# importZL/semantic_segmentation

Hardware: AMD Instinct MI355X
Metric: images/sec (fwd+bwd) U-Net 256x256 bs=32 per GPU (higher is better)
Workload: dtype f16; 1 GPU; unet.UNet(1,2) 256x256 fwd+bwd, CE+Dice loss, batch 32/GPU (BASELINE configs[1]); global_batch=32, parallelism=dp1, dice=per-rank

## Files before the change

include/gsseg.h:

```cpp
#ifndef GSSEG_H
#define GSSEG_H

#include <stdint.h>

#ifdef __cplusplus
extern "C" {
#endif

#define GS_ABI_VERSION 52

enum GsDtype { GS_F16 = 0, GS_BF16 = 1 };
enum GsStatus { GS_OK = 0, GS_EINVAL = -1, GS_ELAUNCH = -2, GS_EUNSUPPORTED = -3 };
enum GsAct { GS_ACT_NONE = 0, GS_ACT_RELU = 1, GS_ACT_LEAKY02 = 2, GS_ACT_TANH = 3 };

#define GS_MAX_TAPS 64

typedef struct GsConvGeom {
    int32_t N, IH, IW, Cin, in_pix_stride, in_coff;
    int32_t OHg, OWg, Cout;
    int32_t OH, OW, out_pix_stride, out_coff;
    int32_t isy, isx, osy, osx, ooy, oox;
    int32_t ntaps;
    int32_t tap_dy[GS_MAX_TAPS], tap_dx[GS_MAX_TAPS];
    int32_t tap_w[GS_MAX_TAPS];
    int32_t Dg, Din, Dout, isz, osz, ooz;
    int32_t tap_dz[GS_MAX_TAPS];
} GsConvGeom;

const char* gs_last_error(void);
int gs_abi_version(void);

int gs_conv_igemm_mtiles(const GsConvGeom* g);
// ... 100 lines not shown
                     int res_pix_stride, int res_coff, void* dz, int NB, int D, int H, int W, int C, int dtype,
                     void* stream);

int gs_maxpool2x2_fwd(const void* z, int z_pix_stride, int z_coff, void* zp, int N, int H, int W, int C, int dtype,
                      void* stream);
int gs_maxpool2x2_fwd_pair(const void* z_hi, const void* z_lo, int z_pix_stride, void* zp_hi, void* zp_lo, int zp_pix_stride, int N, int H,
                           int W, int C, int dtype, void* stream);

int gs_colsum(const void* t, int pix_stride, int coff, int N, int H, int W, int y0, int x0, int h, int w, int C,
              float gscale, float* ws, float* out, int dtype, void* stream);

int gs_head1x1_bn_fwd(const void* y_conv, const float* bn_scale, const float* bn_shift, int act, const float* w,
                      const float* bias, float* logits, int N, int H, int W, int Cout, int dtype, void* stream);
int gs_head1x1_bn_wgrad(const void* y_conv, const float* bn_scale, const float* bn_shift, int act, const float* w,
                        const float* dl, float* dw, float* db, float* ws, int N, int H, int W, int Cout, float gscale,
                        int dtype, void* stream);

int gs_bn_act_bwd_reduce_head(const void* y, const float* dl, const float* w_head, int ncls, const float* scale,
                              const float* shift, const float* mean, const float* invstd, int act, float* partials, int N,
                              int H, int W, int C, int dtype, void* stream);
int gs_bn_act_bwd_apply_head(const void* y, const float* dl, const float* w_head, int ncls, const float* scale,
                             const float* shift, const float* mean, const float* invstd, const float* c1, const float* c2,
                             int act, void* dy, int N, int H, int W, int C, int dtype, void* stream);

int gs_bn_partials_colsum(const float* partials, int ntiles, int Cfull, int coff, int C, float gscale, float* out,
                          void* stream);

int gs_pack_weight(const float* w, void* w_fwd, void* w_dgrad, int Cout, int Cin, int taps, int transposed,
                   int dtype, void* stream);

typedef struct GsPackDesc {
    const float* w;
    void* w_fwd;
    void* w_dgrad;
    int32_t Cout, Cin, taps, transposed;
} GsPackDesc;
int gs_pack_weight_multi(int n, const GsPackDesc* descs, int dtype, void* stream);
int gs_unpack_wgrad(const float* dw, float* grad, int A, int B, int taps, int transposed, float gscale, void* stream);

int64_t gs_fake_postprocess_ws_floats(int N);
int gs_fake_postprocess(const float* x, float* out, float* ws, const float* gamma_lut, int N, int64_t hw, void* stream);

int64_t gs_isic_fake_trans_ws_bytes(int planes, int64_t hw);
int gs_isic_fake_trans(const float* x, float* out, void* ws, int N, int C, int H, int W, int equalize_on, int bits,
                       int sharpness_on, float sharp_r1, float sharp_r2, int autocontrast_on, int saturation_on, float sat_r1,
                       float sat_r2, void* stream);
// ... 165 lines not shown
```

semantic_segmentation_amd/_lib.py:

```python
from __future__ import annotations

import ctypes
import os
import subprocess
from ctypes import POINTER, c_char_p, c_double, c_float, c_int, c_int32, c_int64, c_void_p

_HERE = os.path.dirname(os.path.abspath(__file__))
LIB_PATH = os.environ.get("GSSEG_LIB", os.path.join(_HERE, "libgsseg_hip.so"))
CSRC = os.path.join(_HERE, "csrc")

GS_F16, GS_BF16 = 0, 1
ACT_NONE, ACT_RELU, ACT_LEAKY02, ACT_TANH = 0, 1, 2, 3
GS_MAX_TAPS = 64
ABI_VERSION = 52


class GsConvGeom(ctypes.Structure):
    _fields_ = [(n, c_int32) for n in (
        "N", "IH", "IW", "Cin", "in_pix_stride", "in_coff", "OHg", "OWg", "Cout", "OH", "OW",
        "out_pix_stride", "out_coff", "isy", "isx", "osy", "osx", "ooy", "oox", "ntaps")] + [
        ("tap_dy", c_int32 * GS_MAX_TAPS), ("tap_dx", c_int32 * GS_MAX_TAPS), ("tap_w", c_int32 * GS_MAX_TAPS)] + [
        (n, c_int32) for n in ("Dg", "Din", "Dout", "isz", "osz", "ooz")] + [("tap_dz", c_int32 * GS_MAX_TAPS)]


class GsPackDesc(ctypes.Structure):
    _fields_ = [("w", c_void_p), ("w_fwd", c_void_p), ("w_dgrad", c_void_p)] + [
        (n, c_int32) for n in ("Cout", "Cin", "taps", "transposed")]


GS_SEG_MAX = 4


class GsSegPackDesc(ctypes.Structure):
    _fields_ = [("w", c_void_p), ("pack", c_void_p)] + [(n, c_int32) for n in ("Cout", "Cin", "taps", "transposed", "nseg")] + [
        ("kind", c_int32 * GS_SEG_MAX), ("ci0", c_int32 * GS_SEG_MAX), ("len", c_int32 * GS_SEG_MAX)]


# ... 60 lines not shown
    "gs_bn_bwd_tiles_used": (c_int, [c_int, c_int, c_int, c_int]),
    "gs_bn_act_bwd_reduce": (c_int, [_P, _P, c_int, c_int, _P, _P, c_int, _P, c_float, _F, _F, _F, _F, c_int, _F]
                             + [c_int] * 5 + [c_void_p]),
    "gs_bn_bwd_coeffs": (c_int, [_F, c_int, c_int, c_double, c_float, _F, _F, _F, _F, c_void_p]),
    "gs_bn_act_bwd_apply": (c_int, [_P, _P, c_int, c_int, _P, _P, c_int, _P, c_float, _F, _F, _F, _F, _F, _F, c_int,
                                    c_int, _P]
                            + [c_int] * 5 + [c_void_p]),
    "gs_maxpool3d_fwd": (c_int, [_P, c_int, c_int, _P] + [c_int] * 6 + [c_void_p]),
    "gs_maxpool2x2_fwd": (c_int, [_P, c_int, c_int, _P] + [c_int] * 5 + [c_void_p]),
    "gs_maxpool2x2_fwd_pair": (c_int, [_P, _P, c_int, _P, _P, c_int] + [c_int] * 5 + [c_void_p]),
    "gs_maxpool3d_bwd": (c_int, [_P, c_int, c_int, _P, _P, c_int, c_int, _P] + [c_int] * 6 + [c_void_p]),
    "gs_colsum": (c_int, [_P, c_int, c_int] + [c_int] * 8 + [c_float, _F, _F, c_int, c_void_p]),
    "gs_stem_bn_bwd_wgrad": (c_int, [_P, _P, c_int, c_int, _F, _F, _F, _F, _F, _F, _F, c_int, _F, _F, c_int, c_int, c_int,
                                     c_float, c_int, c_void_p]),
    "gs_stem_stats": (c_int, [_F, _F, _F, _F, c_int, c_int, c_int, c_void_p]),
    "gs_stem_bwd_onepass": (c_int, [_F, _P, _P, c_int, c_int, c_int, _F, _F, c_int, c_int, c_int, c_int, c_void_p]),
    "gs_stem_bwd_finalize": (c_int, [_F, _F, _F, _F, _F, _F, _F, c_int, c_float, _F, _F, _F, c_int, c_int, c_int, c_void_p]),
    "gs_stem_fwd_bn": (c_int, [_F, _F, _F, _F, c_int, _P, c_int, c_int, c_int, c_int, c_void_p]),
    "gs_stem_bwd_tiles": (c_int, [c_int, c_int, c_int]),
    "gs_head1x1_bn_fwd": (c_int, [_P, _F, _F, c_int, _F, _F, _F] + [c_int] * 5 + [c_void_p]),
    "gs_head1x1_bn_wgrad": (c_int, [_P, _F, _F, c_int, _F, _F, _F, _F, _F] + [c_int] * 4 + [c_float, c_int, c_void_p]),
    "gs_bn_act_bwd_reduce_head": (c_int, [_P, _F, _F, c_int, _F, _F, _F, _F, c_int, _F] + [c_int] * 5 + [c_void_p]),
    "gs_bn_act_bwd_apply_head": (c_int, [_P, _F, _F, c_int, _F, _F, _F, _F, _F, _F, c_int, _P] + [c_int] * 5 + [c_void_p]),
    "gs_bn_partials_colsum": (c_int, [_F, c_int, c_int, c_int, c_int, c_float, _F, c_void_p]),
    "gs_pack_weight": (c_int, [_F, _P, _P, c_int, c_int, c_int, c_int, c_int, c_void_p]),
    "gs_pack_weight_multi": (c_int, [c_int, POINTER(GsPackDesc), c_int, c_void_p]),
    "gs_unpack_wgrad": (c_int, [_F, _F, c_int, c_int, c_int, c_int, c_float, c_void_p]),
    "gs_upconv_merge_pack": (c_int, [_F, _F, _F, _F, _P, _P, _F, c_int, c_int, c_int, c_void_p]),
    "gs_fake_postprocess_ws_floats": (c_int64, [c_int]),
    "gs_isic_fake_trans_ws_bytes": (c_int64, [c_int, c_int64]),
    "gs_isic_fake_trans": (c_int, [_F, _F, _P, c_int, c_int, c_int, c_int, c_int, c_int, c_int, c_float, c_float, c_int, c_int,
                                   c_float, c_float, c_void_p]),
    "gs_fake_postprocess": (c_int, [_F, _F, _F, _F, c_int, c_int64, c_void_p]),
    "gs_upconv8_image_fwd": (c_int, [_P, c_int, c_int, _P, c_int, _F, _F, _P] + [c_int] * 7 + [c_void_p]),
    "gs_upconv8_image_wgrad_ok": (c_int, [c_int, c_int]),
    "gs_upconv8_image_wgrad_ws_floats": (c_int64, [c_int] * 4),
    "gs_upconv8_image_wgrad": (c_int, [_P, c_int, _P, c_int, _F, _F] + [c_int] * 5 + [c_void_p]),
    "gs_upconv_split_wgrad": (c_int, [_F, _F, _F, _F, _F, c_float, _F, _F, _F, _F, c_int, c_int, c_void_p]),
    "gs_upconv_split_wgrad_det": (c_int, [_F, _F, _F, _F, _F, c_float, _F, _F, _F, _F, _F, c_int, c_int, c_void_p]),
    "gs_upconv_split_wgrad_ws_floats": (c_int64, [c_int, c_int]),
    "gs_upconv_split_wgrad_parts_ok": (c_int, [c_int, c_int]),
    "gs_upconv_split_wgrad_parts": (c_int, [_F, c_int, c_int64, _F, _F, _F, _F, c_float, _F, _F, _F, _F, _F, c_int, c_int, c_void_p]),
    "gs_nchw_to_nhwc": (c_int, [_F, _P] + [c_int] * 7 + [c_void_p]),
    "gs_nhwc_to_nchw": (c_int, [_P, c_int, c_int, _F] + [c_int] * 4 + [c_float, c_int, c_void_p]),
    "gs_seg_loss_fwd": (c_int, [_F, _P, c_int, c_int, c_int, c_int, _F, _F, c_void_p]),
    "gs_seg_loss_bwd": (c_int, [_F, _P, _F, _F, c_float, _F, c_int, c_int, c_int, c_int, c_void_p]),
# ... 90 lines not shown
```

semantic_segmentation_amd/csrc/bn.hip:

```cpp
#include <stdlib.h>

#include "common.hpp"

namespace {

constexpr int RED_SLICES = 64;

__global__ __launch_bounds__(256) void reduce_partials_stage1(const float* __restrict__ part, int ntiles, int C,
                                                              int tiles_per_slice, double* __restrict__ out1) {
    __shared__ double red[2][8][32];
    const int cl = threadIdx.x & 31, tl = threadIdx.x >> 5;
    const int c = blockIdx.x * 32 + cl;
    const int t0 = blockIdx.y * tiles_per_slice, t1 = min(ntiles, t0 + tiles_per_slice);
    double s1 = 0.0, s2 = 0.0;
    if (c < C) {
        for (int tt = t0 + tl; tt < t1; tt += 8) {
            s1 += (double)part[((int64_t)tt * 2 + 0) * C + c];
            s2 += (double)part[((int64_t)tt * 2 + 1) * C + c];
        }
    }
    red[0][tl][cl] = s1;
    red[1][tl][cl] = s2;
    __syncthreads();
    if (tl == 0 && c < C) {
// ... 43 lines not shown
    shift[c] = bt - (float)mean * sc;
    mean_out[c] = (float)mean;
    invstd_out[c] = invstd;
    if (running_mean) running_mean[c] = (1.f - momentum) * running_mean[c] + momentum * (float)mean;
    if (running_var) {
        const double unb = count > 1.0 ? var * (count / (count - 1.0)) : var;
        running_var[c] = (1.f - momentum) * running_var[c] + momentum * (float)unb;
    }
}

__global__ void bn_eval_coeffs_kernel(int C, const float* gamma, const float* beta, const float* rm, const float* rv,
                                      float eps, float* scale, float* shift, float* mean, float* invstd) {
    const int c = blockIdx.x * blockDim.x + threadIdx.x;
    if (c >= C) return;
    const float is = 1.f / sqrtf(rv[c] + eps);
    const float sc = (gamma ? gamma[c] : 1.f) * is;
    scale[c] = sc;
    shift[c] = (beta ? beta[c] : 0.f) - rm[c] * sc;
    mean[c] = rm[c];
    invstd[c] = is;
}

template <typename T>
__global__ __launch_bounds__(256) void bn_bwd_coeffs_kernel(const T* __restrict__ s, int nslices, int C, double count,
                                                            float gscale, float* dgamma, float* dbeta, float* c1, float* c2) {
    double s1, s2;
    sum_slices_32x8(s, nslices, C, s1, s2);
    const int c = blockIdx.x * 32 + (threadIdx.x & 31);
    if (c >= C || threadIdx.x >= 32) return;
    if (dbeta) dbeta[c] = (float)(s1 * gscale);
    if (dgamma) dgamma[c] = (float)(s2 * gscale);
    c1[c] = (float)(s1 / count);
    c2[c] = (float)(s2 / count);
}

static int bn_traversal() {
    static const int v = getenv("GSSEG_BN_REV") ? atoi(getenv("GSSEG_BN_REV")) : 3;
    return v;
}

struct ApplyArgs {
    const unsigned short* y;
    const float* scale;
    const float* shift;
    unsigned short* z;
    unsigned short* zp;
    const uint8_t* keep;
    float keep_scale;
    int act, N, H, W, C, zs, zc;
    int rev;
};

template <int DT, bool POOL, bool GENERIC>
__global__ __launch_bounds__(256) void bn_act_apply_kernel(const ApplyArgs a) {
    const float slope = a.act == GS_ACT_RELU ? 0.f : (a.act == GS_ACT_LEAKY02 ? 0.2f : 1.f);
    auto fwd_a = [&](float v) __attribute__((always_inline)) { return GENERIC ? act_fwd(v, a.act) : (v > 0.f ? v : v * slope); };
// ... 64 lines not shown
__device__ __forceinline__ float mul_rn(float a, float b) {
    float r;
    asm("v_mul_f32 %0, %1, %2" : "=v"(r) : "v"(a), "v"(b));
    return r;
}

struct BwdArgs {
    const unsigned short* y;
    const unsigned short* dza;
    const unsigned short* dzp;
    const unsigned short* dzb;
    const uint8_t* keep;
    float keep_scale;
    int act_b;
    const float *scale, *shift, *mean, *invstd, *c1, *c2;
    float* partials;
    unsigned short* dy;
    int sa, ca, act, bn, N, H, W, C;
    int tile_units;
    int rev;
    const float* head_dl;
    const float* head_w;
    int head_n;
};

template <int DT, bool POOL, bool APPLY, bool GENERIC, int HEAD = 0, bool EXTRA = true, bool RN = false>
__global__ __launch_bounds__(256) void bn_act_bwd_kernel(const BwdArgs a) {
    static_assert(!HEAD || (!POOL && !GENERIC), "the head source: plain pixels, slope-family activation");
    static_assert(!(RN && GENERIC), "the rounded slope product belongs to the slope family");
    auto mul_g = [&](float g, float d) __attribute__((always_inline)) { return RN ? mul_rn(g, d) : g * d; };
    constexpr int NH = HEAD ? HEAD : 1;
    constexpr int HEAD_CHUNK = 2048;
    __shared__ float hdl[HEAD ? NH * HEAD_CHUNK : 1];
    __shared__ float red[2][256 * 8 / 8][8];
    const float slope_a = a.act == GS_ACT_RELU ? 0.f : (a.act == GS_ACT_LEAKY02 ? 0.2f : 1.f);
    const float slope_b = a.act_b == GS_ACT_RELU ? 0.f : (a.act_b == GS_ACT_LEAKY02 ? 0.2f : 1.f);
    auto grad_a = [&](float v) __attribute__((always_inline)) { return GENERIC ? act_grad(v, a.act) : (v > 0.f ? 1.f : slope_a); };
    auto grad_b = [&](float v) __attribute__((always_inline)) { return GENERIC ? act_grad(v, a.act_b) : (v > 0.f ? 1.f : slope_b); };
    auto fwd_a = [&](float v) __attribute__((always_inline)) { return GENERIC ? act_fwd(v, a.act) : (v > 0.f ? v : v * slope_a); };
    const int nch = a.C >> 3;
    const int PH = POOL ? (a.H + 1) / 2 : a.H, PW = POOL ? (a.W + 1) / 2 : a.W;
    const int units = a.N * PH * PW;
    const int lanes_per_unit = nch < 256 ? nch : 256;
    const int unit_lanes = 256 / lanes_per_unit;
    const int chl = threadIdx.x % lanes_per_unit, ul = threadIdx.x / lanes_per_unit;
    const int tile = a.rev ? (int)(gridDim.x - 1 - blockIdx.x) : (int)blockIdx.x;
    const int u0 = tile * a.tile_units;
    int u1 = u0 + a.tile_units < units ? u0 + a.tile_units : units;
    if (ul >= unit_lanes) u1 = u0;
    constexpr int UNR = 4;

// ... 1 lines not shown
        const bool ch_ok = ch < nch;
        const int c0 = ch_ok ? ch * 8 : 0;
        if (!ch_ok) u1 = u0;
        float sc[8], sh[8], mu[8], is[8], k1[8], k2[8];
#pragma unroll
        for (int i = 0; i < 8; ++i) {
            sc[i] = a.scale ? a.scale[c0 + i] : 1.f;
            sh[i] = a.shift ? a.shift[c0 + i] : 0.f;
            mu[i] = a.mean ? a.mean[c0 + i] : 0.f;
            is[i] = a.invstd ? a.invstd[c0 + i] : 1.f;
            k1[i] = (APPLY && a.c1) ? a.c1[c0 + i] : 0.f;
            k2[i] = (APPLY && a.c2) ? a.c2[c0 + i] : 0.f;
        }
        float s1[8], s2[8];
#pragma unroll
        for (int i = 0; i < 8; ++i) { s1[i] = 0.f; s2[i] = 0.f; }
        float hw[NH][8];
        if (HEAD) {
#pragma unroll
            for (int k = 0; k < NH; ++k)
#pragma unroll
                for (int i = 0; i < 8; ++i) hw[k][i] = k < a.head_n ? a.head_w[k * a.C + c0 + i] : 0.f;
        }
        const int HWp = a.H * a.W;

        if (!POOL) {
            const int tile_end = u0 + a.tile_units < units ? u0 + a.tile_units : units;
            const int chunk = HEAD ? HEAD_CHUNK : (tile_end - u0 > 0 ? tile_end - u0 : 1);
            for (int cb = u0; cb < tile_end; cb += chunk) {
            const int ce = cb + chunk < tile_end ? cb + chunk : tile_end;
            if (HEAD) {
                __syncthreads();
                for (int i = threadIdx.x; i < ce - cb; i += 256) {
                    const int p = cb + i, n = p / HWp, hwp = p - n * HWp;
#pragma unroll
                    for (int q = 0; q < NH; ++q) hdl[q * HEAD_CHUNK + i] = q < a.head_n ? a.head_dl[((int64_t)n * a.head_n + q) * HWp + hwp] : 0.f;
                }
                __syncthreads();
            }
            const int ue = ce < u1 ? ce : u1;
            for (int ub = cb + ul; ub < ue; ub += unit_lanes * UNR) {
                uint4 ry[UNR], rg[UNR], rb[UNR];
                uint2 rk[UNR];
                bool ok[UNR];
                float hd[UNR][NH];
#pragma unroll
// ... 21 lines not shown
                    unpack8<DT>(rg[k], g);
                    unpack8<DT>(rb[k], gb);
                    if (HEAD) {
#pragma unroll
                        for (int i = 0; i < 8; ++i) {
                            float t = hd[k][0] * hw[0][i];
#pragma unroll
                            for (int q = 1; q < NH; ++q) t += hd[k][q] * hw[q][i];
                            g[i] = t;
                        }
                    }
                    if (EXTRA && a.keep) {
                        const unsigned int kw[2] = {rk[k].x, rk[k].y};
#pragma unroll
                        for (int i = 0; i < 8; ++i) g[i] *= ((kw[i >> 2] >> (8 * (i & 3))) & 0xffu) ? a.keep_scale : 0.f;
                    }
#pragma unroll
                    for (int i = 0; i < 8; ++i) {
                        const float v = yv[i] * sc[i] + sh[i];
                        const float gh = mul_g(g[i], grad_a(v)) + ((EXTRA && a.dzb) ? mul_g(gb[i], grad_b(v)) : 0.f);
                        const float xh = (yv[i] - mu[i]) * is[i];
                        if (APPLY) out[i] = a.bn ? sc[i] * (gh - k1[i] - xh * k2[i]) : gh;
                        else { s1[i] += gh; s2[i] += gh * xh; }
                    }
                    if (APPLY) st16(a.dy + pix * a.C + c0, pack8<DT>(out));
                }
            }
            }
        } else {
            const int PH2 = a.H / 2, PW2 = a.W / 2;
            for (int u = u0 + ul; u < u1; u += unit_lanes) {
                const int px = u % PW;
                const int r = u / PW;
                const int py = r % PH;
                const int n = r / PH;
                uint4 ry[4], rg[4];
                bool ok[4];
                int64_t pixk[4];
#pragma unroll
                for (int k = 0; k < 4; ++k) {
                    const int yy = 2 * py + (k >> 1), xx = 2 * px + (k & 1);
                    ok[k] = yy < a.H && xx < a.W;
                    pixk[k] = ((int64_t)n * a.H + (yy < a.H ? yy : a.H - 1)) * a.W + (xx < a.W ? xx : a.W - 1);
                    ry[k] = *reinterpret_cast<const uint4*>(a.y + pixk[k] * a.C + c0);
                    rg[k] = a.dza ? *reinterpret_cast<const uint4*>(a.dza + pixk[k] * a.sa + a.ca + c0) : make_uint4(0, 0, 0, 0);
                }
// ... 37 lines not shown
                        const float v = yv[k][i] * sc[i] + sh[i];
                        const float gh = mul_g(gz, grad_a(v));
                        const float xh = (yv[k][i] - mu[i]) * is[i];
                        if (APPLY) out[i] = a.bn ? sc[i] * (gh - k1[i] - xh * k2[i]) : gh;
                        else { s1[i] += gh; s2[i] += gh * xh; }
                    }
                    if (APPLY) st16(a.dy + pixk[k] * a.C + c0, pack8<DT>(out));
                }
            }
        }
        if (!APPLY) {
            __syncthreads();
#pragma unroll
            for (int i = 0; i < 8; ++i) { red[0][threadIdx.x][i] = s1[i]; red[1][threadIdx.x][i] = s2[i]; }
            __syncthreads();
            const int nv = lanes_per_unit * 8;
            for (int v = threadIdx.x; v < 2 * nv; v += 256) {
                const int st = v >= nv ? 1 : 0, idx = v - st * nv;
                const int cl = idx >> 3, i = idx & 7;
                if (ch - chl + cl >= nch) continue;
                float tsum = 0.f;
                for (int k = 0; k < unit_lanes; ++k) tsum += red[st][k * lanes_per_unit + cl][i];
                a.partials[(int64_t)tile * 2 * a.C + st * a.C + (ch - chl + cl) * 8 + i] = tsum;
            }
        }
    }
}

template <int DT>
__global__ __launch_bounds__(256) void colsum_stage1(const unsigned short* __restrict__ t, int ps, int coff,
                                                     int64_t npix, int C, int64_t pix_per_block, float* ws,
                                                     int H, int W, int y0, int x0, int h, int w) {
    __shared__ float red[256][8];
    const int nch = C >> 3;
    const int lpu = nch < 256 ? nch : 256, ulanes = 256 / lpu;
    const int chl = threadIdx.x % lpu, ul = threadIdx.x / lpu;
    const int64_t p0 = (int64_t)blockIdx.x * pix_per_block;
    int64_t p1 = p0 + pix_per_block < npix ? p0 + pix_per_block : npix;
    if (ul >= ulanes) p1 = p0;
    for (int ch = chl; ch - chl < nch; ch += lpu) {
        float s[8];
#pragma unroll
        for (int i = 0; i < 8; ++i) s[i] = 0.f;
        if (ch >= nch) p1 = p0;
        for (int64_t p = p0 + ul; p < p1; p += ulanes) {
            float v[8];
            const int xx = (int)(p % w);
            const int64_t r = p / w;
            const int yy = (int)(r % h);
            const int64_t n = r / h;
            const int64_t pp = (n * H + y0 + yy) * W + x0 + xx;
            unpack8<DT>(*reinterpret_cast<const uint4*>(t + pp * ps + coff + ch * 8), v);
#pragma unroll
            for (int i = 0; i < 8; ++i) s[i] += v[i];
        }
        __syncthreads();
#pragma unroll
        for (int i = 0; i < 8; ++i) red[threadIdx.x][i] = s[i];
        __syncthreads();
        for (int v = threadIdx.x; v < lpu * 8; v += 256) {
            const int cl = v >> 3, i = v & 7;
            if (ch - chl + cl >= nch) continue;
            float tt = 0.f;
            for (int k = 0; k < ulanes; ++k) tt += red[k * lpu + cl][i];
            ws[(int64_t)blockIdx.x * C + (ch - chl + cl) * 8 + i] = tt;
        }
    }
}
__global__ __launch_bounds__(256) void colsum_stage2(const float* ws, int nblocks, int C, float gscale, float* out) {
    __shared__ double red[8][32];
    const int cl = threadIdx.x & 31, tl = threadIdx.x >> 5;
    const int c = blockIdx.x * 32 + cl;
    double s = 0.0;
    if (c < C) {
        double a[8] = {0, 0, 0, 0, 0, 0, 0, 0};
        int i = tl;
        for (; i + 56 < nblocks; i += 64) {
            float v[8];
#pragma unroll
            for (int u = 0; u < 8; ++u) v[u] = ws[(int64_t)(i + 8 * u) * C + c];
#pragma unroll
            for (int u = 0; u < 8; ++u) a[u] += (double)v[u];
        }
        for (; i < nblocks; i += 8) a[0] += (double)ws[(int64_t)i * C + c];
        s = ((a[0] + a[1]) + (a[2] + a[3])) + ((a[4] + a[5]) + (a[6] + a[7]));
    }
    red[tl][cl] = s;
    __syncthreads();
    if (tl == 0 && c < C) {
        double t = 0.0;
#pragma unroll
        for (int i = 0; i < 8; ++i) t += red[i][cl];
        out[c] = (float)(t * gscale);
    }
}

__global__ __launch_bounds__(256) void partials_colsum_stage1(const float* __restrict__ part, int ntiles, int Cfull, int coff, int C,
                                                              int tiles_per_slice, double* __restrict__ out1) {
    __shared__ double red[8][32];
    const int cl = threadIdx.x & 31, tl = threadIdx.x >> 5;
    const int c = blockIdx.x * 32 + cl;
    const int t0 = blockIdx.y * tiles_per_slice, t1 = min(ntiles, t0 + tiles_per_slice);
    double s1 = 0.0;
    if (c < C)
        for (int tt = t0 + tl; tt < t1; tt += 8) s1 += (double)part[(int64_t)tt * 2 * Cfull + coff + c];
    red[tl][cl] = s1;
    __syncthreads();
    if (tl == 0 && c < C) {
        double a = 0.0;
#pragma unroll
        for (int i = 0; i < 8; ++i) a += red[i][cl];
        out1[(int64_t)blockIdx.y * C + c] = a;
    }
}

template <typename T>
__global__ __launch_bounds__(256) void partials_colsum_final(const T* __restrict__ s, int n, int64_t stride, int C, float gscale,
// ... 126 lines not shown
    const int PH = pool ? (a.H + 1) / 2 : a.H, PW = pool ? (a.W + 1) / 2 : a.W;
    const int64_t units = (int64_t)a.N * PH * PW;
    const int ntiles_max = gs_bn_bwd_tiles(a.N, a.H, a.W);
    a.tile_units = (int)cdiv64(units, ntiles_max);
    if (a.tile_units < 1) a.tile_units = 1;
    const int ntiles = (int)cdiv64(units, a.tile_units);
    if (ntiles_out) *ntiles_out = ntiles;
    const bool generic = a.act == GS_ACT_TANH || (a.dzb && a.act_b == GS_ACT_TANH);
    const bool leaky = !generic && (a.act == GS_ACT_LEAKY02 || (a.dzb && a.act_b == GS_ACT_LEAKY02));
#define LAUNCH(DT, G, R)                                                                                \
    do {                                                                                                \
        if (pool) {                                                                                     \
            if (apply) bn_act_bwd_kernel<DT, true, true, G, 0, true, R><<<ntiles, 256, 0, s>>>(a);      \
            else bn_act_bwd_kernel<DT, true, false, G, 0, true, R><<<ntiles, 256, 0, s>>>(a);           \
        } else if (a.dzb != nullptr || a.keep != nullptr) {                                             \
            if (apply) bn_act_bwd_kernel<DT, false, true, G, 0, true, R><<<ntiles, 256, 0, s>>>(a);     \
            else bn_act_bwd_kernel<DT, false, false, G, 0, true, R><<<ntiles, 256, 0, s>>>(a);          \
        } else {                                                                                        \
            if (apply) bn_act_bwd_kernel<DT, false, true, G, 0, false, R><<<ntiles, 256, 0, s>>>(a);    \
            else bn_act_bwd_kernel<DT, false, false, G, 0, false, R><<<ntiles, 256, 0, s>>>(a);         \
        }                                                                                               \
    } while (0)
    if (a.head_dl != nullptr) {
#define LAUNCH_HEAD(DT, NC, R)                                                                          \
    do {                                                                                                \
        if (apply) bn_act_bwd_kernel<DT, false, true, false, NC, false, R><<<ntiles, 256, 0, s>>>(a);   \
        else bn_act_bwd_kernel<DT, false, false, false, NC, false, R><<<ntiles, 256, 0, s>>>(a);        \
    } while (0)
#define LAUNCH_HEAD_N(DT, R) do { if (a.head_n <= 2) LAUNCH_HEAD(DT, 2, R); else LAUNCH_HEAD(DT, 4, R); } while (0)
        if (dtype == GS_F16) { if (leaky) LAUNCH_HEAD_N(GS_F16, true); else LAUNCH_HEAD_N(GS_F16, false); }
        else { if (leaky) LAUNCH_HEAD_N(GS_BF16, true); else LAUNCH_HEAD_N(GS_BF16, false); }
#undef LAUNCH_HEAD_N
#undef LAUNCH_HEAD
        return 0;
    }
    if (dtype == GS_F16) { if (generic) LAUNCH(GS_F16, true, false); else if (leaky) LAUNCH(GS_F16, false, true); else LAUNCH(GS_F16, false, false); }
    else { if (generic) LAUNCH(GS_BF16, true, false); else if (leaky) LAUNCH(GS_BF16, false, true); else LAUNCH(GS_BF16, false, false); }
#undef LAUNCH
    return 0;
}

extern "C" int gs_bn_bwd_tiles_used(int N, int H, int W, int pooled) {
    const int PH = pooled ? (H + 1) / 2 : H, PW = pooled ? (W + 1) / 2 : W;
    const int64_t units = (int64_t)N * PH * PW;
    const int ntiles_max = gs_bn_bwd_tiles(N, H, W);
    int64_t tu = cdiv64(units, ntiles_max);
    if (tu < 1) tu = 1;
    return (int)cdiv64(units, tu);
}

// ... 65 lines not shown
    GS_CHECK_ARG(dtype == GS_F16 || dtype == GS_BF16, "%s: bad dtype", who);
    GS_CHECK_ARG((int64_t)N * H * W < 2147483647LL, "%s: more than 2^31 pixels", who);
    GS_CHECK_ARG(act == GS_ACT_NONE || act == GS_ACT_RELU || act == GS_ACT_LEAKY02, "%s: activation %d not supported", who, act);
    GS_CHECK_ARG(scale && shift && mean && invstd, "%s: needs the BatchNorm coefficients", who);
    a.y = (const unsigned short*)y; a.head_dl = dl; a.head_w = w_head; a.head_n = ncls;
    a.scale = scale; a.shift = shift; a.mean = mean; a.invstd = invstd; a.act = act; a.bn = 1;
    a.N = N; a.H = H; a.W = W; a.C = C;
    return GS_OK;
}

extern "C" int gs_bn_act_bwd_reduce_head(const void* y, const float* dl, const float* w_head, int ncls, const float* scale,
                                         const float* shift, const float* mean, const float* invstd, int act, float* partials,
                                         int N, int H, int W, int C, int dtype, void* stream) {
    BwdArgs a{};
    int rc = bn_head_args("gs_bn_act_bwd_reduce_head", a, y, dl, w_head, ncls, scale, shift, mean, invstd, act, N, H, W, C, dtype);
    if (rc) return rc;
    GS_CHECK_ARG(partials != nullptr, "gs_bn_act_bwd_reduce_head: null partials");
    a.partials = partials;
    launch_bwd(a, false, dtype, (hipStream_t)stream, nullptr);
    GS_CHECK_LAUNCH("gs_bn_act_bwd_reduce_head");
    return GS_OK;
}

extern "C" int gs_bn_act_bwd_apply_head(const void* y, const float* dl, const float* w_head, int ncls, const float* scale,
                                        const float* shift, const float* mean, const float* invstd, const float* c1,
                                        const float* c2, int act, void* dy, int N, int H, int W, int C, int dtype, void* stream) {
    BwdArgs a{};
    int rc = bn_head_args("gs_bn_act_bwd_apply_head", a, y, dl, w_head, ncls, scale, shift, mean, invstd, act, N, H, W, C, dtype);
    if (rc) return rc;
    GS_CHECK_ARG(dy && c1 && c2, "gs_bn_act_bwd_apply_head: null pointer");
    a.c1 = c1; a.c2 = c2; a.dy = (unsigned short*)dy;
    launch_bwd(a, true, dtype, (hipStream_t)stream, nullptr);
    GS_CHECK_LAUNCH("gs_bn_act_bwd_apply_head");
    return GS_OK;
}

extern "C" int gs_bn_partials_colsum(const float* partials, int ntiles, int Cfull, int coff, int C, float gscale, float* out,
                                     void* stream) {
    GS_CHECK_ARG(partials && out && ntiles > 0 && Cfull > 0 && C > 0 && coff >= 0 && coff + C <= Cfull,
                 "gs_bn_partials_colsum: bad arguments");
    hipStream_t s = (hipStream_t)stream;
    if (ntiles <= direct_tiles()) {
        partials_colsum_final<float><<<cdiv(C, 32), 256, 0, s>>>(partials + coff, ntiles, (int64_t)2 * Cfull, C, gscale, out);
    } else {
        int slices = ntiles < RED_SLICES ? ntiles : RED_SLICES;
        const int tps = cdiv(ntiles, slices);
// ... 29 lines not shown
```

semantic_segmentation_amd/ops.py:

```python
from __future__ import annotations

import collections
import ctypes
import os
from typing import List, Optional, Sequence, Tuple

import torch

from . import _lib
from ._lib import ACT_NONE, GS_BF16, GS_F16, GsConvGeom

DTYPES = {"f16": (GS_F16, torch.float16), "bf16": (GS_BF16, torch.bfloat16)}


def dt_code(t: torch.Tensor) -> int:
    if t.dtype == torch.float16:
        return GS_F16
    if t.dtype == torch.bfloat16:
        return GS_BF16
    raise TypeError(f"expected a float16/bfloat16 tensor, got {t.dtype}")


def _p(t: Optional[torch.Tensor]):
    return None if t is None else t.data_ptr()
# ... 783 lines not shown
              ncls, float(gscale), dt_code(y_conv), _stream())


def bn_act_bwd_reduce_head(y, dl, w_head, scale, shift, mean, invstd, act, partials):
    _dev(y)
    _f32(dl, "dl"); _f32(w_head, "w_head"); _f32(partials, "partials")
    N, H, W, C = y.shape
    ncls = dl.shape[1]
    if tuple(dl.shape) != (N, ncls, H, W) or w_head.numel() != ncls * C or not (dl.is_contiguous() and w_head.is_contiguous()):
        raise ValueError("bn_act_bwd_reduce_head: dl [N,ncls,H,W] and w_head [ncls,C] contiguous fp32")
    _lib.call("gs_bn_act_bwd_reduce_head", _p(y), _p(dl), _p(w_head), ncls, _p(scale), _p(shift), _p(mean), _p(invstd), act,
              _p(partials), N, H, W, C, dt_code(y), _stream())


def bn_act_bwd_apply_head(y, dl, w_head, scale, shift, mean, invstd, c1, c2, act, dy):
    _dev(y)
    _f32(dl, "dl"); _f32(w_head, "w_head")
    N, H, W, C = y.shape
    ncls = dl.shape[1]
    if tuple(dl.shape) != (N, ncls, H, W) or w_head.numel() != ncls * C or not (dl.is_contiguous() and w_head.is_contiguous()):
        raise ValueError("bn_act_bwd_apply_head: dl [N,ncls,H,W] and w_head [ncls,C] contiguous fp32")
    _lib.call("gs_bn_act_bwd_apply_head", _p(y), _p(dl), _p(w_head), ncls, _p(scale), _p(shift), _p(mean), _p(invstd),
              _p(c1), _p(c2), act, _p(dy), N, H, W, C, dt_code(y), _stream())


def bn_partials_colsum(partials, ntiles, Cfull, coff, C, gscale, out):
    _f32(partials, "partials"); _f32(out, "out")
    if partials.numel() < bn_partials_numel(ntiles, Cfull) or out.numel() < C:
        raise ValueError("bn_partials_colsum: buffer too small")
    _lib.call("gs_bn_partials_colsum", _p(partials), ntiles, Cfull, coff, C, float(gscale), _p(out), _stream())


def colsum(t, pix_stride, coff, N, H, W, y0, x0, h, w, C, gscale, ws, out):
    _f32(ws, "ws"); _f32(out, "out")
    if ws.numel() < 1024 * C:
        raise ValueError("colsum: workspace must hold 1024*C floats")
    _lib.call("gs_colsum", _p(t), pix_stride, coff, N, H, W, y0, x0, h, w, C, float(gscale), _p(ws), _p(out),
              dt_code(t), _stream())


def pack_weight(w, w_fwd, w_dgrad, transposed: bool):
    _dev(w)
    _f32(w, "weight")
    if transposed:
        Cin, Cout = w.shape[0], w.shape[1]
    else:
# ... 564 lines not shown
```

semantic_segmentation_amd/unet/unet_engine.py:

```python
from __future__ import annotations

import functools
import math
import os
import warnings
from typing import Callable, Dict, List, Optional

import torch

from .. import ops
from .._lib import ACT_NONE, ACT_RELU
from ..engine_common import ParamIndex, _flush_nbt, bn_coeffs, compute_dtype, pack_key, pack_reuse_allowed

FOLD_BN_INFERENCE = os.environ.get("GSSEG_FOLD_BN", "1") != "0"
WGRAD_SIDE_STREAM = os.environ.get("GSSEG_WGRAD_STREAM", "0") != "0"
FUSED_STEM_BWD = os.environ.get("GSSEG_STEM_BWD_FUSED", "1") != "0"
FUSED_STEM_FWD = os.environ.get("GSSEG_STEM_FWD_FUSED", "1") != "0"
FUSED_HEAD_FWD = os.environ.get("GSSEG_HEAD_FWD_FUSED", "1") != "0"
FUSED_HEAD_BWD = os.environ.get("GSSEG_HEAD_BWD_FUSED", "1") != "0"
FUSED_UP_BIAS_GRAD = os.environ.get("GSSEG_UP_BIAS_FUSED", "1") != "0"


class _ConvRec:
    __slots__ = ("name", "wkey", "bnkey", "inp", "inp_is_image", "y", "coef", "geom", "cin", "cout", "h", "w",
                 "wd", "train_stats", "inp_stride", "z", "tap_sums", "wide")


class _UpRec:
    __slots__ = ("name", "zin", "cat", "geom_bwd", "geom_wg", "wd", "cin", "cout", "h", "w", "H2", "W2", "pt", "pl")


STREAM_SMALL_CONV = os.environ.get("GSSEG_STREAM_CONV", "1") != "0"


@functools.lru_cache(maxsize=4096)
def stream_conv(N, h, w, cin, cout):
    M = N * h * w
    if not STREAM_SMALL_CONV or M > 8192 or cin % 64 or cout % 32:
        return False
    tiles = (-(-w // 32)) * (-(-h // 8)) if w >= 24 else (-(-w // 16)) * (-(-h // 16))
    if N * tiles * (-(-cout // 64)) > 128:
        return False
# ... 760 lines not shown
        dw_arena = torch.zeros(max(tot_w, 1), dtype=torch.float32, device=dev)
        wg_ws = empty(wg_need, dtype=torch.float32)
        arena_off = [0]

        def dw_take(numel):
            a = arena_off[0]
            arena_off[0] = a + numel
            return dw_arena[a:a + numel]
        npart = 0
        for i in range(5):
            npart = max(npart, ops.bn_partials_numel(ops.bn_bwd_tiles(N, hs[i], ws_[i]), C[i]))
            if i == 0:
                npart = max(npart, ops.bn_partials_numel(ops.stem_bwd_tiles(N, hs[i], ws_[i]), 64))
            if i < 4 and ops.USE_HALO_CONV:
                npart = max(npart, ops.bn_partials_numel(ops.conv3x3_mtiles(N, hs[i], ws_[i], 2 * C[i]), 2 * C[i]))
                if N * hs[i] * ws_[i] <= 8192:
                    npart = max(npart, ops.bn_partials_numel(-(-(N * hs[i] * ws_[i]) // 16), 2 * C[i]))
        partials = empty(npart, dtype=torch.float32)
        col_ws = empty(1024 * 1024, dtype=torch.float32)

        z_last = ctx["z_last"]
        dl = (dlogits.contiguous().float() * S)
        wout = params["outc.conv.weight"]
        dwo = galloc("outc.conv.weight", wout, zero=True)
        dbo = galloc("outc.conv.bias", params["outc.conv.bias"], zero=True)
        head_src = None
        wout_c = wout.detach().contiguous()
        rlast = recs["up4.conv.3"]
        if z_last is None:
            ops.head1x1_bn_wgrad(rlast.y, rlast.coef[0], rlast.coef[1], ACT_RELU, wout_c, dl, dwo, dbo, gscale=inv_s)
        if FUSED_HEAD_BWD and wout.shape[0] <= 4 and dl.is_contiguous():
            head_src = (dl, wout_c)
            dz = None
            if z_last is not None:
                ops.conv_smallcout_bwd(z_last, wout_c, dl, None, dwo, dbo, gscale=inv_s)
        elif 4 < wout.shape[0] <= 64:
            dz = empty(N, H, W, 64)
            ops.head1x1_wide_bwd(z_last, wout_c.reshape(wout.shape[0], 64), dl, dz, dwo, dbo, gscale=inv_s)
        elif wout.shape[0] > 64:
            dzs = torch.zeros((N, H, W, 64), dtype=torch.float32, device=dev)
            for g0 in range(0, wout.shape[0], 4):
                g1 = min(g0 + 4, wout.shape[0])
                dzg = empty(N, H, W, 64)
                ops.conv_smallcout_bwd(z_last, wout_c[g0:g1].contiguous(), dl[:, g0:g1].contiguous(), dzg, dwo[g0:g1], dbo[g0:g1],
                                       gscale=inv_s)
                dzs += dzg
            dz = dzs.to(tdt)
        else:
            dz = empty(N, H, W, 64)
            if z_last is not None:
                ops.conv_smallcout_bwd(z_last, wout_c, dl, dz, dwo, dbo, gscale=inv_s)
            else:
                ops.conv_smallcout_bwd(None, wout_c, dl, dz, None, None)
        emit("outc.conv.weight", dwo)
        emit("outc.conv.bias", dbo)

        def conv_stage_bwd(rec: _ConvRec, dz_a, sa, ca, dzp, need_dinp: bool, colsum=None, head=None):
            h, w, cin, cout = rec.h, rec.w, rec.cin, rec.cout
            coef = rec.coef
            pooled = dzp is not None
            if rec.y is None:
                wst = params[rec.wkey].detach().contiguous()
                done = False
                if not need_dinp and not pooled and head is None:
                    nts = ops.stem_bwd_tiles(N, h, w)
                    sws = empty(nts * 576, dtype=torch.float32)
                    s1p = empty(nts * 64, dtype=torch.float32)
                    if ops.stem_bwd_onepass(rec.inp, rec.z, dz_a, sa, ca, ACT_RELU, s1p, sws, z_stride=rec.z.shape[3]):
                        dgamma = galloc(rec.bnkey + ".weight", params[rec.bnkey + ".weight"])
                        dbeta = galloc(rec.bnkey + ".bias", params[rec.bnkey + ".bias"])
                        dw = galloc(rec.wkey, params[rec.wkey], zero=True)
                        ops.stem_bwd_finalize(sws, s1p, rec.tap_sums, wst, coef[0], coef[2], coef[3], rec.train_stats, inv_s,
                                              dw, dgamma, dbeta, N, h, w)
                        emit(rec.wkey, dw)
                        emit(rec.bnkey + ".weight", dgamma)
                        emit(rec.bnkey + ".bias", dbeta)
                        done = True
                if done:
                    return None
                y_re = empty(N, h, w, cout)
                ops.conv_smallcin_fwd(rec.inp, wst, None, y_re, None, 3, 1, 1)
                rec.y = y_re
            ntiles = ops.bn_bwd_tiles_used(N, h, w, pooled)
            if head is not None:
                ops.bn_act_bwd_reduce_head(rec.y, head[0], head[1], coef[0], coef[1], coef[2], coef[3], ACT_RELU, partials)
            else:
                ops.bn_act_bwd_reduce(rec.y, dz_a, sa, ca, dzp, coef[0], coef[1], coef[2], coef[3], ACT_RELU, partials)
            dgamma = galloc(rec.bnkey + ".weight", params[rec.bnkey + ".weight"])
            dbeta = galloc(rec.bnkey + ".bias", params[rec.bnkey + ".bias"])
            c12 = empty(2, cout, dtype=torch.float32)
            ops.bn_bwd_coeffs(partials, ntiles, cout, N * h * w, inv_s, dgamma, dbeta, c12[0], c12[1])
            if not rec.train_stats:
                c12.zero_()
            wparam = params[rec.wkey]
            dw_stem = None
            if (rec.inp_is_image and not need_dinp and not pooled and FUSED_STEM_BWD and cin == 1 and cout == 64
                    and rec.inp.is_contiguous()):
                dw_stem = galloc(rec.wkey, wparam, zero=True)
                if ops.stem_bn_bwd_wgrad(rec.y, dz_a, sa, ca, rec.inp, coef[0], coef[1], coef[2], coef[3], c12[0], c12[1],
                                         ACT_RELU, dw_stem, inv_s):
                    emit(rec.wkey, dw_stem)
                    emit(rec.bnkey + ".weight", dgamma)
                    emit(rec.bnkey + ".bias", dbeta)
                    return None
            dy = empty(N, h, w, cout)
            if head is not None:
                ops.bn_act_bwd_apply_head(rec.y, head[0], head[1], coef[0], coef[1], coef[2], coef[3], c12[0], c12[1], ACT_RELU, dy)
            else:
                ops.bn_act_bwd_apply(rec.y, dz_a, sa, ca, dzp, coef[0], coef[1], coef[2], coef[3], c12[0], c12[1],
                                     ACT_RELU, True, dy)
            dinp = None
            if rec.inp_is_image:
                dw = dw_stem if dw_stem is not None else galloc(rec.wkey, wparam, zero=True)
                ops.conv_smallcin_wgrad(rec.inp, dy, dw, 3, 1, 1, inv_s)
# ... 153 lines not shown
```

Measured before the change: 2114 images/sec.

## Fuse output-head weight gradient into the BN backward head reduce pass

```diff
diff --git a/include/gsseg.h b/include/gsseg.h
--- a/include/gsseg.h
+++ b/include/gsseg.h
@@ -7,7 +7,7 @@
 extern "C" {
 #endif
 
-#define GS_ABI_VERSION 52
+#define GS_ABI_VERSION 53
 
 enum GsDtype { GS_F16 = 0, GS_BF16 = 1 };
 enum GsStatus { GS_OK = 0, GS_EINVAL = -1, GS_ELAUNCH = -2, GS_EUNSUPPORTED = -3 };
@@ -154,6 +154,13 @@
 int gs_bn_act_bwd_apply_head(const void* y, const float* dl, const float* w_head, int ncls, const float* scale,
                              const float* shift, const float* mean, const float* invstd, const float* c1, const float* c2,
                              int act, void* dy, int N, int H, int W, int C, int dtype, void* stream);
+
+int64_t gs_bn_head_wgrad_ws_floats(int N, int H, int W, int C, int ncls);
+int gs_bn_act_bwd_reduce_head_wgrad(const void* y, const float* dl, const float* w_head, int ncls, const float* scale,
+                                    const float* shift, const float* mean, const float* invstd, int act, float* partials,
+                                    float* head_ws, int N, int H, int W, int C, int dtype, void* stream);
+int gs_bn_bwd_coeffs_head(const float* partials, int ntiles, int C, double count, float gscale, float* dgamma, float* dbeta,
+                          float* c1, float* c2, const float* head_ws, int ncls, float* dw, float* db, void* stream);
 
 int gs_bn_partials_colsum(const float* partials, int ntiles, int Cfull, int coff, int C, float gscale, float* out,
                           void* stream);
diff --git a/semantic_segmentation_amd/_lib.py b/semantic_segmentation_amd/_lib.py
--- a/semantic_segmentation_amd/_lib.py
+++ b/semantic_segmentation_amd/_lib.py
@@ -12,7 +12,7 @@
 GS_F16, GS_BF16 = 0, 1
 ACT_NONE, ACT_RELU, ACT_LEAKY02, ACT_TANH = 0, 1, 2, 3
 GS_MAX_TAPS = 64
-ABI_VERSION = 52
+ABI_VERSION = 53
 
 
 class GsConvGeom(ctypes.Structure):
@@ -119,6 +119,9 @@
     "gs_head1x1_bn_wgrad": (c_int, [_P, _F, _F, c_int, _F, _F, _F, _F, _F] + [c_int] * 4 + [c_float, c_int, c_void_p]),
     "gs_bn_act_bwd_reduce_head": (c_int, [_P, _F, _F, c_int, _F, _F, _F, _F, c_int, _F] + [c_int] * 5 + [c_void_p]),
     "gs_bn_act_bwd_apply_head": (c_int, [_P, _F, _F, c_int, _F, _F, _F, _F, _F, _F, c_int, _P] + [c_int] * 5 + [c_void_p]),
+    "gs_bn_head_wgrad_ws_floats": (c_int64, [c_int] * 5),
+    "gs_bn_act_bwd_reduce_head_wgrad": (c_int, [_P, _F, _F, c_int, _F, _F, _F, _F, c_int, _F, _F] + [c_int] * 5 + [c_void_p]),
+    "gs_bn_bwd_coeffs_head": (c_int, [_F, c_int, c_int, c_double, c_float, _F, _F, _F, _F, _F, c_int, _F, _F, c_void_p]),
     "gs_bn_partials_colsum": (c_int, [_F, c_int, c_int, c_int, c_int, c_float, _F, c_void_p]),
     "gs_pack_weight": (c_int, [_F, _P, _P, c_int, c_int, c_int, c_int, c_int, c_void_p]),
     "gs_pack_weight_multi": (c_int, [c_int, POINTER(GsPackDesc), c_int, c_void_p]),
diff --git a/semantic_segmentation_amd/csrc/bn.hip b/semantic_segmentation_amd/csrc/bn.hip
--- a/semantic_segmentation_amd/csrc/bn.hip
+++ b/semantic_segmentation_amd/csrc/bn.hip
@@ -89,8 +89,8 @@
 }
 
 template <typename T>
-__global__ __launch_bounds__(256) void bn_bwd_coeffs_kernel(const T* __restrict__ s, int nslices, int C, double count,
-                                                            float gscale, float* dgamma, float* dbeta, float* c1, float* c2) {
+__device__ __forceinline__ void bwd_coeffs_body(const T* __restrict__ s, int nslices, int C, double count, float gscale,
+                                                float* dgamma, float* dbeta, float* c1, float* c2) {
     double s1, s2;
     sum_slices_32x8(s, nslices, C, s1, s2);
     const int c = blockIdx.x * 32 + (threadIdx.x & 31);
@@ -99,6 +99,57 @@
     if (dgamma) dgamma[c] = (float)(s2 * gscale);
     c1[c] = (float)(s1 / count);
     c2[c] = (float)(s2 / count);
+}
+
+template <typename T>
+__global__ __launch_bounds__(256) void bn_bwd_coeffs_kernel(const T* __restrict__ s, int nslices, int C, double count,
+                                                            float gscale, float* dgamma, float* dbeta, float* c1, float* c2) {
+    bwd_coeffs_body(s, nslices, C, count, gscale, dgamma, dbeta, c1, c2);
+}
+
+__device__ __forceinline__ double sum_rows_32x8(const float* __restrict__ ws, int nrows, int64_t stride, int c, bool c_ok) {
+    __shared__ double red[8][32];
+    const int cl = threadIdx.x & 31, tl = threadIdx.x >> 5;
+    double s = 0.0;
+    if (c_ok) {
+        double a[8] = {0, 0, 0, 0, 0, 0, 0, 0};
+        int i = tl;
+        for (; i + 56 < nrows; i += 64) {
+            float v[8];
+#pragma unroll
+            for (int u = 0; u < 8; ++u) v[u] = ws[(int64_t)(i + 8 * u) * stride + c];
+#pragma unroll
+            for (int u = 0; u < 8; ++u) a[u] += (double)v[u];
+        }
+        for (; i < nrows; i += 8) a[0] += (double)ws[(int64_t)i * stride + c];
+        s = ((a[0] + a[1]) + (a[2] + a[3])) + ((a[4] + a[5]) + (a[6] + a[7]));
+    }
+    red[tl][cl] = s;
+    __syncthreads();
+    double t = 0.0;
+    if (tl == 0) {
+#pragma unroll
+        for (int i = 0; i < 8; ++i) t += red[i][cl];
+    }
+    return t;
+}
+
+template <typename T>
+__global__ __launch_bounds__(256) void bn_bwd_coeffs_head_kernel(const T* __restrict__ s, int nslices, int C, double count,
+                                                                 float gscale, float* dgamma, float* dbeta, float* c1, float* c2,
+                                                                 const float* __restrict__ hws, int ntiles, int row, int n, int ndw,
+                                                                 float* dw, float* db) {
+    const int nbn = (C + 31) / 32;
+    if ((int)blockIdx.x < nbn) {
+        bwd_coeffs_body(s, nslices, C, count, gscale, dgamma, dbeta, c1, c2);
+        return;
+    }
+    const int j = ((int)blockIdx.x - nbn) * 32 + (threadIdx.x & 31);
+    const double t = sum_rows_32x8(hws, ntiles, row, j, j < n);
+    if (threadIdx.x < 32 && j < n) {
+        if (j < ndw) dw[j] = (float)(t * gscale);
+        else if (db) db[j - ndw] = (float)(t * gscale);
+    }
 }
 
 static int bn_traversal() {
@@ -209,11 +260,13 @@
     const float* head_dl;
     const float* head_w;
     int head_n;
+    float* head_ws;
 };
 
-template <int DT, bool POOL, bool APPLY, bool GENERIC, int HEAD = 0, bool EXTRA = true, bool RN = false>
+template <int DT, bool POOL, bool APPLY, bool GENERIC, int HEAD = 0, bool EXTRA = true, bool RN = false, bool WG = false>
 __global__ __launch_bounds__(256) void bn_act_bwd_kernel(const BwdArgs a) {
     static_assert(!HEAD || (!POOL && !GENERIC), "the head source: plain pixels, slope-family activation");
+    static_assert(!WG || (HEAD && !APPLY), "the head's weight gradient rides on the head-source reduce");
     static_assert(!(RN && GENERIC), "the rounded slope product belongs to the slope family");
     auto mul_g = [&](float g, float d) __attribute__((always_inline)) { return RN ? mul_rn(g, d) : g * d; };
     constexpr int NH = HEAD ? HEAD : 1;
@@ -261,6 +314,13 @@
 #pragma unroll
                 for (int i = 0; i < 8; ++i) hw[k][i] = k < a.head_n ? a.head_w[k * a.C + c0 + i] : 0.f;
         }
+        float wacc[WG ? NH : 1][8], wsb[WG ? NH : 1];
+#pragma unroll
+        for (int k = 0; k < (WG ? NH : 1); ++k) {
+            wsb[k] = 0.f;
+#pragma unroll
+            for (int i = 0; i < 8; ++i) wacc[k][i] = 0.f;
+        }
         const int HWp = a.H * a.W;
 
         if (!POOL) {
@@ -328,6 +388,15 @@
                         const float xh = (yv[i] - mu[i]) * is[i];
                         if (APPLY) out[i] = a.bn ? sc[i] * (gh - k1[i] - xh * k2[i]) : gh;
                         else { s1[i] += gh; s2[i] += gh * xh; }
+                        if (WG) {
+                            const float z = fwd_a(v);
+#pragma unroll
+                            for (int q = 0; q < NH; ++q) wacc[q][i] += hd[k][q] * z;
+                        }
+                    }
+                    if (WG) {
+#pragma unroll
+                        for (int q = 0; q < NH; ++q) wsb[q] += hd[k][q];
                     }
                     if (APPLY) st16(a.dy + pix * a.C + c0, pack8<DT>(out));
                 }
@@ -411,6 +480,38 @@
                 float tsum = 0.f;
                 for (int k = 0; k < unit_lanes; ++k) tsum += red[st][k * lanes_per_unit + cl][i];
                 a.partials[(int64_t)tile * 2 * a.C + st * a.C + (ch - chl + cl) * 8 + i] = tsum;
+            }
+        }
+        if (WG) {
+            const int nv = lanes_per_unit * 8;
+            float* wrow = a.head_ws + (int64_t)tile * (a.head_n * a.C + 4);
+#pragma unroll
+            for (int q = 0; q < NH; q += 2) {
+                __syncthreads();
+#pragma unroll
+                for (int i = 0; i < 8; ++i) { red[0][threadIdx.x][i] = wacc[q][i]; red[1][threadIdx.x][i] = wacc[q + 1][i]; }
+                __syncthreads();
+                for (int v = threadIdx.x; v < 2 * nv; v += 256) {
+                    const int st = v >= nv ? 1 : 0, idx = v - st * nv;
+                    const int cl = idx >> 3, i = idx & 7;
+                    if (ch - chl + cl >= nch || q + st >= a.head_n) continue;
+                    float tsum = 0.f;
+                    for (int k = 0; k < unit_lanes; ++k) tsum += red[st][k * lanes_per_unit + cl][i];
+                    wrow[(q + st) * a.C + (ch - chl + cl) * 8 + i] = tsum;
+                }
+            }
+            if (ch == chl) {
+                __syncthreads();
+                if (chl == 0) {
+#pragma unroll
+                    for (int q = 0; q < NH; ++q) red[0][ul][q] = wsb[q];
+                }
+                __syncthreads();
+                if ((int)threadIdx.x < a.head_n) {
+                    float tsum = 0.f;
+                    for (int k = 0; k < unit_lanes; ++k) tsum += red[0][k][threadIdx.x];
+                    wrow[a.head_n * a.C + threadIdx.x] = tsum;
+                }
             }
         }
     }
@@ -457,31 +558,9 @@
     }
 }
 __global__ __launch_bounds__(256) void colsum_stage2(const float* ws, int nblocks, int C, float gscale, float* out) {
-    __shared__ double red[8][32];
-    const int cl = threadIdx.x & 31, tl = threadIdx.x >> 5;
-    const int c = blockIdx.x * 32 + cl;
-    double s = 0.0;
-    if (c < C) {
-        double a[8] = {0, 0, 0, 0, 0, 0, 0, 0};
-        int i = tl;
-        for (; i + 56 < nblocks; i += 64) {
-            float v[8];
-#pragma unroll
-            for (int u = 0; u < 8; ++u) v[u] = ws[(int64_t)(i + 8 * u) * C + c];
-#pragma unroll
-            for (int u = 0; u < 8; ++u) a[u] += (double)v[u];
-        }
-        for (; i < nblocks; i += 8) a[0] += (double)ws[(int64_t)i * C + c];
-        s = ((a[0] + a[1]) + (a[2] + a[3])) + ((a[4] + a[5]) + (a[6] + a[7]));
-    }
-    red[tl][cl] = s;
-    __syncthreads();
-    if (tl == 0 && c < C) {
-        double t = 0.0;
-#pragma unroll
-        for (int i = 0; i < 8; ++i) t += red[i][cl];
-        out[c] = (float)(t * gscale);
-    }
+    const int c = blockIdx.x * 32 + (threadIdx.x & 31);
+    const double t = sum_rows_32x8(ws, nblocks, C, c, c < C);
+    if (threadIdx.x < 32 && c < C) out[c] = (float)(t * gscale);
 }
 
 __global__ __launch_bounds__(256) void partials_colsum_stage1(const float* __restrict__ part, int ntiles, int Cfull, int coff, int C,
@@ -654,10 +733,11 @@
         }                                                                                               \
     } while (0)
     if (a.head_dl != nullptr) {
-#define LAUNCH_HEAD(DT, NC, R)                                                                          \
-    do {                                                                                                \
-        if (apply) bn_act_bwd_kernel<DT, false, true, false, NC, false, R><<<ntiles, 256, 0, s>>>(a);   \
-        else bn_act_bwd_kernel<DT, false, false, false, NC, false, R><<<ntiles, 256, 0, s>>>(a);        \
+#define LAUNCH_HEAD(DT, NC, R)                                                                                  \
+    do {                                                                                                        \
+        if (apply) bn_act_bwd_kernel<DT, false, true, false, NC, false, R><<<ntiles, 256, 0, s>>>(a);           \
+        else if (a.head_ws) bn_act_bwd_kernel<DT, false, false, false, NC, false, R, true><<<ntiles, 256, 0, s>>>(a); \
+        else bn_act_bwd_kernel<DT, false, false, false, NC, false, R><<<ntiles, 256, 0, s>>>(a);                \
     } while (0)
 #define LAUNCH_HEAD_N(DT, R) do { if (a.head_n <= 2) LAUNCH_HEAD(DT, 2, R); else LAUNCH_HEAD(DT, 4, R); } while (0)
         if (dtype == GS_F16) { if (leaky) LAUNCH_HEAD_N(GS_F16, true); else LAUNCH_HEAD_N(GS_F16, false); }
@@ -769,6 +849,47 @@
     return GS_OK;
 }
 
+extern "C" int64_t gs_bn_head_wgrad_ws_floats(int N, int H, int W, int C, int ncls) {
+    if (N <= 0 || H <= 0 || W <= 0 || C <= 0 || ncls < 1 || ncls > 4) return 0;
+    return (int64_t)gs_bn_bwd_tiles(N, H, W) * ((int64_t)ncls * C + 4);
+}
+
+extern "C" int gs_bn_act_bwd_reduce_head_wgrad(const void* y, const float* dl, const float* w_head, int ncls, const float* scale,
+                                               const float* shift, const float* mean, const float* invstd, int act,
+                                               float* partials, float* head_ws, int N, int H, int W, int C, int dtype,
+                                               void* stream) {
+    BwdArgs a{};
+    int rc = bn_head_args("gs_bn_act_bwd_reduce_head_wgrad", a, y, dl, w_head, ncls, scale, shift, mean, invstd, act, N, H, W, C, dtype);
+    if (rc) return rc;
+    GS_CHECK_ARG(partials != nullptr && head_ws != nullptr, "gs_bn_act_bwd_reduce_head_wgrad: null partials / head_ws");
+    a.partials = partials;
+    a.head_ws = head_ws;
+    launch_bwd(a, false, dtype, (hipStream_t)stream, nullptr);
+    GS_CHECK_LAUNCH("gs_bn_act_bwd_reduce_head_wgrad");
+    return GS_OK;
+}
+
+extern "C" int gs_bn_bwd_coeffs_head(const float* partials, int ntiles, int C, double count, float gscale, float* dgamma,
+                                     float* dbeta, float* c1, float* c2, const float* head_ws, int ncls, float* dw, float* db,
+                                     void* stream) {
+    GS_CHECK_ARG(partials && c1 && c2 && ntiles > 0 && C > 0 && count > 0, "gs_bn_bwd_coeffs_head: bad arguments");
+    GS_CHECK_ARG(head_ws && dw && ncls >= 1 && ncls <= 4, "gs_bn_bwd_coeffs_head: needs head_ws, dw and 1..4 classes");
+    hipStream_t s = (hipStream_t)stream;
+    const int ndw = ncls * C, n = ndw + ncls, row = ndw + 4;
+    const int blocks = cdiv(C, 32) + cdiv(n, 32);
+    if (ntiles <= direct_tiles()) {
+        bn_bwd_coeffs_head_kernel<float><<<blocks, 256, 0, s>>>(partials, ntiles, C, count, gscale, dgamma, dbeta, c1, c2,
+                                                                 head_ws, ntiles, row, n, ndw, dw, db);
+    } else {
+        double* o1; int ns;
+        reduce_partials(partials, ntiles, C, &o1, &ns, s);
+        bn_bwd_coeffs_head_kernel<double><<<blocks, 256, 0, s>>>(o1, ns, C, count, gscale, dgamma, dbeta, c1, c2,
+                                                                  head_ws, ntiles, row, n, ndw, dw, db);
+    }
+    GS_CHECK_LAUNCH("gs_bn_bwd_coeffs_head");
+    return GS_OK;
+}
+
 extern "C" int gs_bn_act_bwd_apply_head(const void* y, const float* dl, const float* w_head, int ncls, const float* scale,
                                         const float* shift, const float* mean, const float* invstd, const float* c1,
                                         const float* c2, int act, void* dy, int N, int H, int W, int C, int dtype, void* stream) {
diff --git a/semantic_segmentation_amd/ops.py b/semantic_segmentation_amd/ops.py
--- a/semantic_segmentation_amd/ops.py
+++ b/semantic_segmentation_amd/ops.py
@@ -829,6 +829,31 @@
         raise ValueError("bn_act_bwd_apply_head: dl [N,ncls,H,W] and w_head [ncls,C] contiguous fp32")
     _lib.call("gs_bn_act_bwd_apply_head", _p(y), _p(dl), _p(w_head), ncls, _p(scale), _p(shift), _p(mean), _p(invstd),
               _p(c1), _p(c2), act, _p(dy), N, H, W, C, dt_code(y), _stream())
+
+
+def bn_head_wgrad_ws(N, H, W, C, ncls, device):
+    return torch.empty(int(_lib.load().gs_bn_head_wgrad_ws_floats(N, H, W, C, ncls)), dtype=torch.float32, device=device)
+
+
+def bn_act_bwd_reduce_head_wgrad(y, dl, w_head, scale, shift, mean, invstd, act, partials, head_ws):
+    _dev(y)
+    _f32(dl, "dl"); _f32(w_head, "w_head"); _f32(partials, "partials"); _f32(head_ws, "head_ws")
+    N, H, W, C = y.shape
+    ncls = dl.shape[1]
+    if tuple(dl.shape) != (N, ncls, H, W) or w_head.numel() != ncls * C or not (dl.is_contiguous() and w_head.is_contiguous()):
+        raise ValueError("bn_act_bwd_reduce_head_wgrad: dl [N,ncls,H,W] and w_head [ncls,C] contiguous fp32")
+    if head_ws.numel() < _lib.load().gs_bn_head_wgrad_ws_floats(N, H, W, C, ncls) or partials.numel() < bn_partials_numel(bn_bwd_tiles(N, H, W), C):
+        raise ValueError("bn_act_bwd_reduce_head_wgrad: partials / head_ws too small")
+    _lib.call("gs_bn_act_bwd_reduce_head_wgrad", _p(y), _p(dl), _p(w_head), ncls, _p(scale), _p(shift), _p(mean), _p(invstd), act,
+              _p(partials), _p(head_ws), N, H, W, C, dt_code(y), _stream())
+
+
+def bn_bwd_coeffs_head(partials, ntiles, C, count, gscale, dgamma, dbeta, c1, c2, head_ws, ncls, dw, db):
+    _f32(partials, "partials"); _f32(head_ws, "head_ws"); _f32(dw, "dw"); _f32(db, "db")
+    if head_ws.numel() < ntiles * (ncls * C + 4) or dw.numel() != ncls * C or db.numel() != ncls or not (dw.is_contiguous() and db.is_contiguous()):
+        raise ValueError("bn_bwd_coeffs_head: head_ws [ntiles, ncls*C+4], dw [ncls,C], db [ncls] contiguous fp32")
+    _lib.call("gs_bn_bwd_coeffs_head", _p(partials), ntiles, C, float(count), float(gscale), _p(dgamma), _p(dbeta), _p(c1), _p(c2),
+              _p(head_ws), ncls, _p(dw), _p(db), _stream())
 
 
 def bn_partials_colsum(partials, ntiles, Cfull, coff, C, gscale, out):
diff --git a/semantic_segmentation_amd/unet/unet_engine.py b/semantic_segmentation_amd/unet/unet_engine.py
--- a/semantic_segmentation_amd/unet/unet_engine.py
+++ b/semantic_segmentation_amd/unet/unet_engine.py
@@ -18,6 +18,7 @@
 FUSED_STEM_FWD = os.environ.get("GSSEG_STEM_FWD_FUSED", "1") != "0"
 FUSED_HEAD_FWD = os.environ.get("GSSEG_HEAD_FWD_FUSED", "1") != "0"
 FUSED_HEAD_BWD = os.environ.get("GSSEG_HEAD_BWD_FUSED", "1") != "0"
+FUSED_HEAD_WGRAD = os.environ.get("GSSEG_HEAD_WGRAD_FUSED", "1") != "0"
 FUSED_UP_BIAS_GRAD = os.environ.get("GSSEG_UP_BIAS_FUSED", "1") != "0"
 
 
@@ -824,15 +825,16 @@
         z_last = ctx["z_last"]
         dl = (dlogits.contiguous().float() * S)
         wout = params["outc.conv.weight"]
-        dwo = galloc("outc.conv.weight", wout, zero=True)
-        dbo = galloc("outc.conv.bias", params["outc.conv.bias"], zero=True)
+        head_wgrad = (z_last is None and FUSED_HEAD_BWD and FUSED_HEAD_WGRAD and wout.shape[0] <= 4 and dl.is_contiguous())
+        dwo = galloc("outc.conv.weight", wout, zero=not head_wgrad)
+        dbo = galloc("outc.conv.bias", params["outc.conv.bias"], zero=not head_wgrad)
         head_src = None
         wout_c = wout.detach().contiguous()
         rlast = recs["up4.conv.3"]
-        if z_last is None:
+        if z_last is None and not head_wgrad:
             ops.head1x1_bn_wgrad(rlast.y, rlast.coef[0], rlast.coef[1], ACT_RELU, wout_c, dl, dwo, dbo, gscale=inv_s)
         if FUSED_HEAD_BWD and wout.shape[0] <= 4 and dl.is_contiguous():
-            head_src = (dl, wout_c)
+            head_src = (dl, wout_c, dwo, dbo) if head_wgrad else (dl, wout_c)
             dz = None
             if z_last is not None:
                 ops.conv_smallcout_bwd(z_last, wout_c, dl, None, dwo, dbo, gscale=inv_s)
@@ -854,8 +856,9 @@
                 ops.conv_smallcout_bwd(z_last, wout_c, dl, dz, dwo, dbo, gscale=inv_s)
             else:
                 ops.conv_smallcout_bwd(None, wout_c, dl, dz, None, None)
-        emit("outc.conv.weight", dwo)
-        emit("outc.conv.bias", dbo)
+        if not head_wgrad:
+            emit("outc.conv.weight", dwo)
+            emit("outc.conv.bias", dbo)
 
         def conv_stage_bwd(rec: _ConvRec, dz_a, sa, ca, dzp, need_dinp: bool, colsum=None, head=None):
             h, w, cin, cout = rec.h, rec.w, rec.cin, rec.cout
@@ -884,14 +887,25 @@
                 ops.conv_smallcin_fwd(rec.inp, wst, None, y_re, None, 3, 1, 1)
                 rec.y = y_re
             ntiles = ops.bn_bwd_tiles_used(N, h, w, pooled)
-            if head is not None:
+            head_ws = None
+            if head is not None and len(head) == 4:
+                head_ws = ops.bn_head_wgrad_ws(N, h, w, cout, head[0].shape[1], dev)
+                ops.bn_act_bwd_reduce_head_wgrad(rec.y, head[0], head[1], coef[0], coef[1], coef[2], coef[3], ACT_RELU, partials,
+                                                 head_ws)
+            elif head is not None:
                 ops.bn_act_bwd_reduce_head(rec.y, head[0], head[1], coef[0], coef[1], coef[2], coef[3], ACT_RELU, partials)
             else:
                 ops.bn_act_bwd_reduce(rec.y, dz_a, sa, ca, dzp, coef[0], coef[1], coef[2], coef[3], ACT_RELU, partials)
             dgamma = galloc(rec.bnkey + ".weight", params[rec.bnkey + ".weight"])
             dbeta = galloc(rec.bnkey + ".bias", params[rec.bnkey + ".bias"])
             c12 = empty(2, cout, dtype=torch.float32)
-            ops.bn_bwd_coeffs(partials, ntiles, cout, N * h * w, inv_s, dgamma, dbeta, c12[0], c12[1])
+            if head_ws is not None:
+                ops.bn_bwd_coeffs_head(partials, ntiles, cout, N * h * w, inv_s, dgamma, dbeta, c12[0], c12[1], head_ws,
+                                       head[0].shape[1], head[2], head[3])
+                emit("outc.conv.weight", head[2])
+                emit("outc.conv.bias", head[3])
+            else:
+                ops.bn_bwd_coeffs(partials, ntiles, cout, N * h * w, inv_s, dgamma, dbeta, c12[0], c12[1])
             if not rec.train_stats:
                 c12.zero_()
             wparam = params[rec.wkey]
```

Result: no change. 2124 images/sec, median of 6 (+0.5%).
